# polarlightman/Scoring-rules-for-Gaussian-process-regression-a-new-approach-to-inference

Hardware: AMD Instinct MI355X
Metric: GP fit+predict+CRPS wall-clock (ms) at n=20k full / n=40k FITC; HBM GB/s & MFMA% (higher is better)
Workload: dtype f64; 1 GPU; C3 full GP fit(NLML+LOO-CRPS+LOO-LogS)+predict+score; n=20000, d=8, n_test=5000, kernel=ARD, parallelism=single

## Files before the change

include/gpscore.h:

```cpp
#ifndef GPSCORE_H
#define GPSCORE_H

#include <stdint.h>

#ifdef __cplusplus
extern "C" {
#endif

typedef struct gps_ctx gps_ctx;

enum { GPS_ARD = 0, GPS_RBF = 1 };
enum { GPS_FULL = 0, GPS_LOWER = 1 };

enum {
  GPS_OBJ_NLML = 0,
  GPS_OBJ_LOO_CRPS = 1,
  GPS_OBJ_LOO_LOGS = 2,
  GPS_OBJ_LOGDET = 3,
  GPS_OBJ_QUAD = 4,
  GPS_N_OBJ = 5
};
enum {
  GPS_SC_CRPS = 0, GPS_SC_LOGS = 1, GPS_SC_MSLL = 2, GPS_SC_SMSE = 3,
  GPS_SC_MSE = 4, GPS_SC_COVER = 5, GPS_N_SC = 6
// ... 13 lines not shown
  GPS_OPT_OVERLAP = 0,
  GPS_OPT_GEMM_MAP = 3,
  GPS_OPT_TINY_GEMM = 7,
  GPS_OPT_GRAM_REG = 9,
  GPS_OPT_GRAPH = 10,
  GPS_OPT_PRED_PRE = 11,
  GPS_OPT_DAG = 12,
  GPS_OPT_AR_CHUNKS = 15,
  GPS_OPT_DAG_TILES = 13,
  GPS_OPT_STREAM_K = 18,
  GPS_OPT_DAG_WGS = 19,
  GPS_OPT_DAG_GROUP = 17,
  GPS_OPT_SLAB_XCD = 26,
  GPS_OPT_DAG_ORDER = 25,
  GPS_OPT_FITC_DEP = 27,
};
int gps_ctx_set_option(gps_ctx* ctx, int key, int value);

enum { GPS_STAT_GRAPHS = 0, GPS_STAT_GRAPH_CAP = 1, GPS_STAT_GRAPH_OVERFLOW = 2,
       GPS_STAT_DEVICE_BYTES = 3, GPS_STAT_GRAPH_DROPPED = 4, GPS_STAT_GRAPH_EVICTED = 5,
       GPS_N_STATS = 6 };
int gps_ctx_stats(gps_ctx* ctx, int64_t* out, int cap);

int gps_dag_task_list(int T, int flags, uint32_t* out, int cap);

typedef struct gps_gemm_desc {
  int32_t lay_a, lay_b, epi;
  int32_t M, N, K;
  int64_t lda, ldb, ldc;
  double alpha, beta;
  int32_t tri, tri_off;
  int32_t lower_out, mirror;
  int32_t kend;
  int32_t tile, ksplit, map_mode;
  int32_t use_ws, sk_alone, dep_mode;
  int32_t reserved;
  int64_t ld_out, c_kslice_stride;
} gps_gemm_desc;
enum { GPS_GEMM_PLAN_TILE = 0, GPS_GEMM_PLAN_KSPLIT = 1, GPS_GEMM_PLAN_MAP = 2,
// ... 178 lines not shown
```

scoring-rules-for-gaussian-process-regression-a-new-approach-to-inference_amd/csrc/api.hip:

```cpp
#include "api_internal.h"

namespace gpsapi {

thread_local std::string g_err;

int fail(gps_ctx* ctx, int code, const std::string& msg) {
  if (ctx) ctx->err = msg;
  g_err = msg;
  return code;
}

hipError_t sync_ctx_streams(gps_ctx* ctx) {
  for (hipStream_t st : {ctx->stream, ctx->side, ctx->aux[0], ctx->aux[1]})
    if (st) {
      const hipError_t e = hipStreamSynchronize(st);
      if (e != hipSuccess) return e;
    }
  return hipSuccess;
}

hipError_t drop_graphs_in(gps_ctx* ctx, const void* p, size_t bytes) {
  if (!ctx || !p || ctx->pgraphs.empty()) return hipSuccess;
  const uintptr_t lo = (uintptr_t)p, hi = lo + bytes;
  bool synced = false;
// ... 200 lines not shown

int fitc_rowsq_dep(gps_ctx* ctx, const double* L, int* sig, int64_t ncols, int mode,
                   hipStream_t st, int64_t nb_dag) {
  const int64_t np = ctx->fn_pad, mp = ctx->m_pad;
  GemmParams p = gp0();
  p.A = ctx->Knm.d(); p.lda = mp; p.B = L; p.ldb = mp;
  p.M = (int)np; p.N = (int)ncols; p.K = (int)ncols; p.tri = TRI_K_LE_J;
  p.kend = (int)pad_to(ctx->m, 16);
  p.out0 = ctx->fslab.d(); p.ld_out = np;
  p.dep_sig = sig; p.dep_q = sig + kSigQueue; p.dep_err = static_cast<int*>(ctx->info.p) + 1;
  p.dep_grid = dag_width(ctx, nb_dag, true); p.dep_mode = mode;
  return gemm(ctx, LAY_N, LAY_T, EPI_ROWSQ, p, st);
}

int dag_list_key(const gps_ctx* ctx, int64_t nb) {
  return (int)(3 * nb + ctx->dag_order);
}

bool dag_block(const gps_ctx* ctx, int64_t nb) { return ctx->dag && nb >= 2 && nb <= ctx->dag_tiles; }

void dag_blocks(const gps_ctx* ctx, int64_t nb, std::vector<int>& sizes, int64_t& cnt) {
  if (nb <= 1) return;
  if (dag_block(ctx, nb)) {
    sizes.push_back((int)nb);
    cnt += dag_cnt_ints((int)nb);
    return;
  }
  dag_blocks(ctx, nb / 2, sizes, cnt);
  dag_blocks(ctx, nb - nb / 2, sizes, cnt);
}

int dag_width(const gps_ctx* ctx, int64_t nb, bool half) {
  const int auto_w = half ? std::max(4, ctx->ncu / 2) : ctx->ncu;
  return (int)std::min<int64_t>(ctx->dag_wgs > 0 ? ctx->dag_wgs : auto_w, std::max<int64_t>(4, 2 * nb * nb));
// ... 9 lines not shown
    ++ctx->fplan.leaves;
    return 0;
  }
  if (dag_block(ctx, nb)) {
    auto it = ctx->dag_lists.find(dag_list_key(ctx, nb));
    const int64_t need = dag_cnt_ints(nb);
    if (it == ctx->dag_lists.end() || ctx->dag_cnt_used + need > (int64_t)(ctx->dag_cnt.cap / 4))
      return fail(ctx, -2, "persistent factorisation: task list / counters not prepared");
    DagParams d;
    d.A = A; d.lda = lda; d.Linv = Linv; d.ldl = ldl; d.Lout = Lout; d.ldlo = ldlo;
    d.logdiag = logdiag; d.info = info; d.base = base; d.nreal = nreal; d.T = nb;
    d.tasks = static_cast<const uint32_t*>(it->second.first.p); d.ntasks = it->second.second;
    d.cnt = static_cast<int*>(ctx->dag_cnt.p) + ctx->dag_cnt_used;
    d.spin_ticks = 200000000ull;
    d.group = ctx->dag_group;
    d.sig = ctx->dag_sig;
    ctx->dag_sig = nullptr;
    ctx->dag_cnt_used += need;
    const double nn = 128.0 * nb;
    Prof pr(ctx, "potrf_dag", 2.0 * nn * nn * nn / 3.0, 0);
    HIPCHK(launch_potrf_dag(d, dag_width(ctx, nb, ctx->dag_half), s));
    gps_ctx::FactorPlan& fp = ctx->fplan;
    fp.dag_tmin = fp.dags ? std::min(fp.dag_tmin, nb) : nb;
    fp.dag_tmax = std::max(fp.dag_tmax, nb);
    ++fp.dags;
    return 0;
  }
  const int n1b = nb / 2, n2b = nb - n1b;
  const int n1 = n1b * GPS_TILE, n2 = n2b * GPS_TILE;
  double* A21 = A + (int64_t)n1 * lda;
// ... 115 lines not shown
bool factor_zeroed(const gps_ctx* ctx, const double* p, int64_t n_pad) {
  const auto it = ctx->zeroed.find((uintptr_t)p);
  return it != ctx->zeroed.end() && it->second == n_pad;
}

int potrf_inv(gps_ctx* ctx, double* A, int64_t n_pad, double* Linv, double* W, double* logdiag,
              int nreal, double* Lout) {
  if (!factor_zeroed(ctx, Linv, n_pad) || (Lout && !factor_zeroed(ctx, Lout, n_pad)))
    return fail(ctx, -1, "potrf_inv: factor buffer not zeroed for this size (internal contract)");
  std::vector<int> dsizes;
  int64_t dcnt = 0;
  dag_blocks(ctx, n_pad / GPS_TILE, dsizes, dcnt);
  for (int T : dsizes) {
    const int lk = dag_list_key(ctx, T);
    if (ctx->dag_lists.count(lk)) continue;
    const std::vector<uint32_t> tl = dag_task_list(T, ctx->dag_order, true);
    auto& e = ctx->dag_lists[lk];
    HIPCHK(ensure(ctx, e.first, tl.size() * 4));
    HIPCHK(hipMemcpyAsync(e.first.p, tl.data(), tl.size() * 4, hipMemcpyHostToDevice, ctx->stream));
    HIPCHK(hipStreamSynchronize(ctx->stream));
    e.second = (int)tl.size();
  }
  if (dcnt && ctx->dag_cnt.cap < (size_t)dcnt * 4) {
    HIPCHK(hipStreamSynchronize(ctx->stream));
    HIPCHK(ensure(ctx, ctx->dag_cnt, std::max<size_t>((size_t)dcnt * 4, (size_t)1 << 20)));
    HIPCHK(hipMemsetAsync(ctx->dag_cnt.p, 0, ctx->dag_cnt.cap, ctx->stream));
    HIPCHK(hipStreamSynchronize(ctx->stream));
  }
  auto eager = [&]() {
    ctx->sync_used = 0;
    ctx->pre.join = nullptr;
// ... 3 lines not shown
                         static_cast<int*>(ctx->info.p), 0, nreal, Lout, n_pad, true);
  };
  if (!ctx->graphs || ctx->prof || n_pad <= GPS_TILE) return eager();
  HIPCHK(ensure(ctx, ctx->ws_main, (size_t)kSplitWsDoubles * 8));
  HIPCHK(ensure(ctx, ctx->ws_side, (size_t)kSplitWsDoubles * 8));
  const bool pre = ctx->pre.kind == PRE_FITC_Q;
  std::vector<uintptr_t> key = {
      (uintptr_t)A, (uintptr_t)n_pad, (uintptr_t)Linv, (uintptr_t)W, (uintptr_t)logdiag,
      (uintptr_t)nreal, (uintptr_t)Lout, (uintptr_t)ctx->stream, (uintptr_t)ctx->side,
      (uintptr_t)ctx->overlap, (uintptr_t)ctx->gemm_map,
      (uintptr_t)g_tiny_gemm, (uintptr_t)g_stream_k, (uintptr_t)g_slab_xcd, (uintptr_t)ctx->info.p, (uintptr_t)ctx->ws_main.p,
      (uintptr_t)ctx->ws_side.p, (uintptr_t)pre,
      pre ? (uintptr_t)ctx->pre.n1 : 0, pre ? (uintptr_t)ctx->aux[0] : 0,
      pre ? (uintptr_t)ctx->Knm.p : 0, pre ? (uintptr_t)ctx->fslab.p : 0,
      pre ? (uintptr_t)ctx->fn_pad : 0, pre ? (uintptr_t)ctx->m_pad : 0, pre ? (uintptr_t)ctx->pre.sig : 0,
      (uintptr_t)ctx->dag, (uintptr_t)ctx->dag_tiles, (uintptr_t)ctx->dag_group, (uintptr_t)ctx->dag_wgs, (uintptr_t)ctx->dag_half,
      (uintptr_t)ctx->dag_cnt.p, (uintptr_t)ctx->sk_cnt.p, (uintptr_t)ctx->dag_sig};
  for (int T : dsizes) key.push_back((uintptr_t)ctx->dag_lists[dag_list_key(ctx, T)].first.p);
  for (auto& g : ctx->pgraphs)
    if (g.key == key) {
      g.last_use = ++ctx->graph_tick;
      HIPCHK(hipGraphLaunch(g.exec, ctx->stream));
      ctx->fplan = g.plan;
      ctx->fplan.replayed = 1;
      return 0;
    }
  if (ctx->pgraphs.size() >= kMaxGraphs) {
    size_t lru = 0;
    for (size_t i = 1; i < ctx->pgraphs.size(); ++i)
      if (ctx->pgraphs[i].last_use < ctx->pgraphs[lru].last_use) lru = i;
    HIPCHK(sync_ctx_streams(ctx));
// ... 225 lines not shown
      ctx->dag_wgs = value;
      return 0;
    case GPS_OPT_FITC_DEP: ctx->fitc_dep = value != 0; return 0;
    case GPS_OPT_DAG_ORDER:
      ARGCHK(value >= 0 && value <= 2, "GPS_OPT_DAG_ORDER must be 0, 1 or 2");
      ctx->dag_order = value;
      return 0;
    case GPS_OPT_DAG_GROUP:
      ARGCHK(value >= 2 && value <= 4, "GPS_OPT_DAG_GROUP must be 2, 3 or 4");
      ctx->dag_group = value;
      return 0;
    case GPS_OPT_DAG_TILES:
      ARGCHK(value >= 2 && value <= 64, "GPS_OPT_DAG_TILES must be in 2..64");
      ctx->dag_tiles = value;
      return 0;
    default: return fail(ctx, -1, "unknown option");
  }
}

void* gps_ctx_stream(gps_ctx* ctx) { return ctx ? (void*)ctx->stream : nullptr; }

int gps_ctx_synchronize(gps_ctx* ctx) {
  if (int rc = bind(ctx)) return rc;
  HIPCHK(hipStreamSynchronize(ctx->stream));
  return 0;
}

int gps_ctx_stats(gps_ctx* ctx, int64_t* out, int cap) {
  if (int rc = bind(ctx)) return rc;
  ARGCHK(out != nullptr && cap >= 0, "out is NULL or cap < 0");
  size_t bytes = 0;
  for (DBuf* b : ctx_buffers(ctx)) bytes += b->cap;
  int64_t v[GPS_N_STATS];
  v[GPS_STAT_GRAPHS] = (int64_t)ctx->pgraphs.size();
  v[GPS_STAT_GRAPH_CAP] = (int64_t)kMaxGraphs;
  v[GPS_STAT_GRAPH_OVERFLOW] = ctx->graph_overflow;
  v[GPS_STAT_GRAPH_DROPPED] = ctx->graph_dropped;
  v[GPS_STAT_GRAPH_EVICTED] = ctx->graph_evicted;
  v[GPS_STAT_DEVICE_BYTES] = (int64_t)bytes;
  for (int i = 0; i < cap && i < GPS_N_STATS; ++i) out[i] = v[i];
  return GPS_N_STATS;
}

int gps_dag_task_list(int T, int flags, uint32_t* out, int cap) {
  if (T < 2 || T > 64 || cap < 0 || (cap > 0 && !out) || (flags & ~13))
    return fail(nullptr, -1, "bad arguments");
  const std::vector<uint32_t> tl = dag_task_list(T, (flags >> 2 & 3) == 0 ? 1 : (flags >> 2 & 3) == 3 ? 0 : flags >> 2 & 3,
                                                 (flags & 1) != 0);
  for (int i = 0; i < cap && i < (int)tl.size(); ++i) out[i] = tl[i];
  return (int)tl.size();
}

int gps_phase_enable(gps_ctx* ctx, int on) {
  if (int rc = bind(ctx)) return rc;
  ctx->phase = on != 0;
  return 0;
}

int gps_phase_collect(gps_ctx* ctx, char* json_out, int64_t cap) {
  if (int rc = bind(ctx)) return rc;
  HIPCHK(sync_ctx_streams(ctx));
  std::map<std::string, std::pair<int, double>> agg;
  std::vector<std::string> order;
// ... 252 lines not shown
```

scoring-rules-for-gaussian-process-regression-a-new-approach-to-inference_amd/csrc/api_full.hip:

```cpp
#include "api_internal.h"

extern "C" {

int gps_full_set_data(gps_ctx* ctx, const double* X, const double* y, int64_t n, int d) {
  if (int rc = bind(ctx)) return rc;
  ARGCHK(X && y && n > 1 && d >= 1 && d <= GPS_MAX_D, "bad training data");
  ARGCHK(n <= (int64_t)1 << 30, "n too large");
  if (d != ctx->d) ctx->have_test = false;
  ctx->n = n;
  ctx->d = d;
  ctx->n_pad = pad_to(n);
  if (int rc = upload(ctx, ctx->X, X, n, d, ctx->n_pad)) return rc;
  if (int rc = upload(ctx, ctx->y, y, n, 1, ctx->n_pad)) return rc;
  double s = 0, s2 = 0;
  for (int64_t i = 0; i < n; ++i) s += y[i];
  const double mean = s / n;
  for (int64_t i = 0; i < n; ++i) s2 += (y[i] - mean) * (y[i] - mean);
  ctx->ytr_mean = mean;
  ctx->ytr_var = s2 / (n - 1);
  ctx->have_data = true;
  ctx->fitted = false;
  HIPCHK(hipStreamSynchronize(ctx->stream));
  return 0;
}
// ... 28 lines not shown
  }
  HIPCHK(ensure(ctx, ctx->W, potrf_ws_doubles(np) * 8));
  HIPCHK(ensure(ctx, ctx->logdiag, np * 8));
  HIPCHK(ensure(ctx, ctx->beta, np * 8));
  HIPCHK(ensure(ctx, ctx->alpha, np * 8));
  HIPCHK(ensure(ctx, ctx->dinv, np * 8));
  HIPCHK(ensure(ctx, ctx->mu_loo, np * 8));
  HIPCHK(ensure(ctx, ctx->var_loo, np * 8));
  const int64_t nchunk = (np + 255) / 256;
  HIPCHK(ensure(ctx, ctx->slab, (size_t)nchunk * np * 2 * 8));
  int rc;
  if ((rc = reset_info(ctx))) return rc;
  if ((rc = gram(ctx, "gram_kff", ctx->X.d(), (int)n, ctx->X.d(), (int)n, ctx->d, ctx->th,
                 ctx->th.sn2, 1, 1, ctx->A.d(), np, (int)np, (int)np)))
    return rc;
  if ((rc = potrf_inv(ctx, ctx->A.d(), np, ctx->Linv.d(), ctx->W.d(), ctx->logdiag.d(), (int)n,
                      nullptr)))
    return rc;
  {
    Prof pr(ctx, "gemv_beta", 0, 4.0 * (double)np * np);
    HIPCHK(launch_gemv_lower(ctx->Linv.d(), np, ctx->y.d(), ctx->beta.d(), (int)np, s));
  }
  int nchunk_c = 0;
  {
    Prof pr(ctx, "colred_alpha_dinv", 0, 4.0 * (double)np * np);
    nchunk_c = launch_colred_partials(ctx->Linv.d(), np, (int)np, (int)np, 1, ctx->beta.d(),
                                      ctx->slab.d(), s);
    ARGCHK(nchunk_c > 0, "column pass launch failed");
  }
  {
    double* part = row_part(ctx, np, 4);
    ARGCHK(part != nullptr, "out of device memory");
    Prof pr(ctx, "loo_finalize", 0, 0);
// ... 214 lines not shown
```

scoring-rules-for-gaussian-process-regression-a-new-approach-to-inference_amd/csrc/api_internal.h:

```cpp
#pragma once
#include <dlfcn.h>
#include <rccl/rccl.h>
#include <stdio.h>
#include <string.h>

#include <chrono>
#include <climits>
#include <cmath>
#include <condition_variable>
#include <map>
#include <memory>
#include <mutex>
#include <string>
#include <vector>

#include "gps_internal.h"
#include "gpscore.h"

using namespace gps;

namespace gpsapi {


struct DBuf {
// ... 66 lines not shown
  hipStream_t aux[2] = {nullptr, nullptr};
  bool overlap = true;
  int gemm_map = 0;
  int ar_chunks = 4;
  std::vector<hipEvent_t> ar_ev;
  int ncu = 0;
  std::vector<hipEvent_t> sync_ev;
  size_t sync_used = 0;
  bool graphs = true;
  bool pred_pre = true;
  bool dag = true;
  int dag_tiles = 20;
  int dag_group = 3;
  int dag_wgs = 0;
  int dag_order = 1;
  bool dag_half = false;
  bool fitc_dep = true;
  int* dag_sig = nullptr;
  DBuf dsig;
  std::map<int, std::pair<DBuf, int>> dag_lists;
  std::map<uintptr_t, int64_t> zeroed;
  DBuf dag_cnt;
  DBuf sk_cnt;
  int64_t dag_cnt_used = 0;
  struct PrePass {
    int kind = 0;
    int64_t n1 = 0;
    const double* L = nullptr;
    hipEvent_t join = nullptr;
    int* sig = nullptr;
// ... 139 lines not shown
void phase_mark(gps_ctx* c, const char* name);
hipEvent_t sync_event(gps_ctx* c);
GemmParams gp0();
const char* gemm_tag(int al, int bl, int epi, const GemmParams& p);
double gemm_flops(const GemmParams& p);
int gemm(gps_ctx* ctx, int al, int bl, int epi, const GemmParams& p, hipStream_t st = nullptr,
         GemmLaunchInfo* info = nullptr);
int gram(gps_ctx* ctx, const char* tag, const double* x, int n, const double* xp, int m, int d,
         const Theta& th, double diag_add, int lower, int pad_identity, double* out, int64_t ldo,
         int M, int N, hipStream_t st = nullptr);
int pred_rows(gps_ctx* ctx, int64_t r0, int64_t r1, const double* w, hipStream_t st);
int fitc_rowsq_cols(gps_ctx* ctx, const double* Lx, int64_t c0, int64_t c1, hipStream_t st);
int fitc_rowsq_dep(gps_ctx* ctx, const double* L, int* sig, int64_t ncols, int mode,
                   hipStream_t st, int64_t nb_dag);
int dag_list_key(const gps_ctx* ctx, int64_t nb);
bool dag_block(const gps_ctx* ctx, int64_t nb);
void dag_blocks(const gps_ctx* ctx, int64_t nb, std::vector<int>& sizes, int64_t& cnt);
int dag_width(const gps_ctx* ctx, int64_t nb, bool half);
int potrf_inv_rec(gps_ctx* ctx, double* A, int64_t lda, double* Linv, int64_t ldl, double* W,
                  int nb, double* logdiag, int* info, int base, int nreal, double* Lout,
                  int64_t ldlo, bool top = false);
size_t potrf_ws_doubles(int64_t n_pad);
int reset_info(gps_ctx* ctx);
hipError_t zero_factor(gps_ctx* ctx, double* p, int64_t n_pad, hipStream_t s);
bool factor_zeroed(const gps_ctx* ctx, const double* p, int64_t n_pad);
int potrf_inv(gps_ctx* ctx, double* A, int64_t n_pad, double* Linv, double* W, double* logdiag,
              int nreal, double* Lout);
int check_info(gps_ctx* ctx);
int set_theta(gps_ctx* ctx, Theta& th, int kind, const double* theta, int n_ell, int d);
int upload(gps_ctx* ctx, DBuf& b, const double* h, int64_t rows, int64_t cols, int64_t rows_pad);
// ... 32 lines not shown
```

scoring-rules-for-gaussian-process-regression-a-new-approach-to-inference_amd/csrc/gps_internal.h:

```cpp
#pragma once

#include <hip/hip_runtime.h>
#include <stdint.h>

#include <string>
#include <vector>

#define GPS_TILE 128
#define GPS_MAX_D 64

namespace gps {

inline int64_t pad_to(int64_t n, int64_t t = GPS_TILE) { return (n + t - 1) / t * t; }

struct GramParams {
  const double* x;
  const double* xp;
  double* out;
  int64_t ldo;
  int n, m;
  int M, N;
  int d;
  double sf2;
  double diag_add;
// ... 287 lines not shown
                             double* Lout, int64_t ldlo, double* logdiag, int* info,
                             int base, int n_real_in_block, hipStream_t s);

struct DagParams {
  double* A; int64_t lda;
  double* Linv; int64_t ldl;
  double* Lout; int64_t ldlo;
  double* logdiag; int* info; int base; int nreal;
  int T;
  const uint32_t* tasks; int ntasks;
  int* cnt;
  unsigned long long spin_ticks;
  unsigned long long* trace = nullptr;
  int group = 3;
  int* sig = nullptr;
};
hipError_t launch_potrf_dag(const DagParams& p, int nwg, hipStream_t s);
std::vector<uint32_t> dag_task_list(int T, int order = 1, bool fine = true);
inline int64_t dag_cnt_ints(int T) { return (16 + 2 * (int64_t)T * T + 63) / 64 * 64; }

hipError_t launch_gemv_lower(const double* L, int64_t ldl, const double* x, double* y,
                             int n_pad, hipStream_t s);
hipError_t launch_gemv_full(const double* M, int64_t ldm, const double* x, double* y,
                            int rows, int cols, hipStream_t s);
hipError_t launch_colred(const double* M, int64_t ldm, int rows, int cols, int lower,
                         const double* w, const double* rowscale, double* s1, double* s2,
                         double* slab, hipStream_t s, int crows = 256);
hipError_t launch_slab_sum(const double* slab, int64_t ld, int nslab, int64_t len,
                           const double* init, double* out, hipStream_t s);
hipError_t launch_sym_slab_sum(const double* slab, int64_t slice_stride, int nslab, int M,
                               const double* base, double* dst, hipStream_t s);

hipError_t launch_sym_pack(const double* slab, int64_t slice_stride, int nslab, int r0, int r1,
// ... 130 lines not shown
```

scoring-rules-for-gaussian-process-regression-a-new-approach-to-inference_amd/csrc/kernels_potrf.hip:

```cpp
#include <algorithm>
#include <queue>
#include <vector>

#include "gps_internal.h"

namespace gps {

namespace v4 {
typedef double d4 __attribute__((ext_vector_type(4)));
typedef double dv2 __attribute__((ext_vector_type(2)));
constexpr int TS = 17;
constexpr int TSZ = 16 * TS;
constexpr int NT = 36;
__device__ __forceinline__ constexpr int tix(int i, int j) { return i * (i + 1) / 2 + j; }

__device__ __forceinline__ double rl(double v, int lane) {
  const int lo = __builtin_amdgcn_readlane(__double2loint(v), lane);
  const int hi = __builtin_amdgcn_readlane(__double2hiint(v), lane);
  return __hiloint2double(hi, lo);
}
template <bool COH>
__device__ __forceinline__ void st_d(double* p, double v) {
  if constexpr (COH)
    __hip_atomic_store(reinterpret_cast<unsigned long long*>(p),
// ... 374 lines not shown
__device__ __forceinline__ double ld64(__amdgpu_buffer_rsrc_t r, uint32_t off) {
  return __builtin_bit_cast(double, __builtin_amdgcn_raw_buffer_load_b64(r, off, 0, AUX_SC1));
}
__device__ __forceinline__ void st64(__amdgpu_buffer_rsrc_t r, uint32_t off, double v) {
  __builtin_amdgcn_raw_buffer_store_b64(__builtin_bit_cast(v2u, v), r, off, 0, AUX_SC1);
}
__device__ __forceinline__ int ld_cnt(const int* p) {
  return __hip_atomic_load(p, __ATOMIC_RELAXED, __HIP_MEMORY_SCOPE_AGENT);
}

template <bool BT, int G>
__device__ __forceinline__ void wave_gemm32(const double* Ap, int64_t lda, const double* Bp,
                                            int64_t ldb, int kb, int ke, d4 (&acc)[2][2]) {
  const int lane = threadIdx.x & 63, r = lane & 15, g = lane >> 4;
  const __amdgpu_buffer_rsrc_t ra = rsrc(Ap, (uint32_t)(32 * lda * 8));
  const __amdgpu_buffer_rsrc_t rb = rsrc(Bp, (uint32_t)((BT ? 32 : 128) * ldb * 8));
  typedef double Frag[G][2][4];
  const int nc = (ke - kb) / 16;
  auto load_group = [&](int c, Frag& a, Frag& b) {
#pragma unroll
    for (int u = 0; u < G; ++u) {
      if (c + u >= nc) break;
      const int k = kb + 16 * (c + u) + 4 * g;
#pragma unroll
      for (int i = 0; i < 2; ++i) {
        const uint32_t oa = (uint32_t)(((int64_t)(16 * i + r) * lda + k) * 8);
        const dv2 a0 = ld128(ra, oa), a1 = ld128(ra, oa + 16);
        a[u][i][0] = a0.x; a[u][i][1] = a0.y; a[u][i][2] = a1.x; a[u][i][3] = a1.y;
        if constexpr (BT) {
          const uint32_t ob = (uint32_t)(((int64_t)(16 * i + r) * ldb + k) * 8);
          const dv2 b0 = ld128(rb, ob), b1 = ld128(rb, ob + 16);
// ... 200 lines not shown
      sh[1] = 0;
      sh[2] = (unsigned int)t;
    }
    __syncthreads();
    const unsigned int w = __builtin_amdgcn_readfirstlane(sh[0]);
    if (w == 0xffffffffu) break;
    if constexpr (TRACE) {
      trow = p.trace + 4 * (int64_t)__builtin_amdgcn_readfirstlane(sh[2]);
      if (tid == 0) {
        unsigned int xcc;
        asm volatile("s_getreg_b32 %0, hwreg(HW_REG_XCC_ID)" : "=s"(xcc));
        trow[0] = __builtin_amdgcn_s_memrealtime();
        trow[3] = (unsigned long long)blockIdx.x << 8 | (xcc & 15);
      }
    }
    const int type = w & 7, part = (w >> 3) & 15, fine = (w >> 7) & 1, ti = (w >> 8) & 255,
              tj = (w >> 16) & 255, tk = (w >> 24) & 255;
    if (wave == 0) {
      const int* c0 = nullptr; const int* c1 = nullptr; const int* c2 = nullptr;
      int v0 = 0, v1 = 0, v2 = 0;
      switch (type) {
        case 0:
          c0 = acnt + ti * T + ti; v0 = U * ti;
          break;
        case 1:
          c0 = acnt + ti * T + tk; v0 = U * tk;
          c1 = xcnt + tk * T + tk; v1 = 1;
          break;
        case 2:
          c0 = acnt + ti * T + tk; v0 = U * (tk + 1);
          c1 = acnt + tj * T + tk; v1 = U * (tk + 1);
          c2 = acnt + ti * T + tj; v2 = U * tk;
          break;
        case 3:
          c0 = acnt + ti * T + tj; v0 = U * (tj + 1);
          c1 = xcnt + tj * T + tk; v1 = tj == tk ? 1 : U * (tj - tk + 1);
          c2 = xcnt + ti * T + tk; v2 = U * (tj - tk);
          break;
        case 4:
          c0 = xcnt + ti * T + tk; v0 = U * (ti - tk);
          c1 = xcnt + ti * T + ti; v1 = 1;
          break;
        default: break;
      }
      if (!c1) { c1 = c0; v1 = v0; }
      if (!c2) { c2 = c0; v2 = v0; }
      constexpr unsigned int kMinPolls = 100000;
      unsigned long long t0 = __builtin_amdgcn_s_memrealtime();
      unsigned int ab = 0, polls = 0;
      int seen = -1;
      for (;;) {
        const int a0 = ld_cnt(c0), a1 = ld_cnt(c1), a2 = ld_cnt(c2), e = ld_cnt(err);
        if (__builtin_amdgcn_readfirstlane((a0 >= v0 && a1 >= v1 && a2 >= v2) ? 1 : 0)) break;
// ... 67 lines not shown
        case 1: {
          const int64_t K = 128 * (int64_t)tk;
          st.A = p.A + (R + q) * lda + K; st.lda = lda;
          st.B = p.Linv + (K + wv) * ldl + K; st.ldb = ldl; st.bt = 1;
          st.C = p.A + (R + q) * lda + K + wv; st.ldc = lda;
          if (p.Lout) { st.C2 = p.Lout + (R + q) * p.ldlo + K + wv; st.ldc2 = p.ldlo; }
          st.alpha = 1.0; st.beta = 0.0; st.kb = 0; st.ke = (int)wv + 32;
          out = acnt + ti * T + tk;
          break;
        }
        case 2: {
          const int64_t J = 128 * (int64_t)tj, K = 128 * (int64_t)tk;
          st.A = p.A + (R + q) * lda + K; st.lda = lda;
          st.B = p.A + (J + wv) * lda + K; st.ldb = lda; st.bt = 1;
          st.C = p.A + (R + q) * lda + J + wv; st.ldc = lda;
          st.alpha = -1.0; st.beta = 1.0; st.kb = 0; st.ke = 128;
          st.active = !(ti == tj && wave > part);
          out = acnt + ti * T + tj;
          break;
        }
        case 3: {
          const int64_t J = 128 * (int64_t)tj, K = 128 * (int64_t)tk;
          st.A = p.A + (R + q) * lda + J; st.lda = lda;
          st.B = p.Linv + J * ldl + K + wv; st.ldb = ldl; st.bt = 0;
          st.C = p.Linv + (R + q) * ldl + K + wv; st.ldc = ldl;
          st.alpha = 1.0; st.beta = tj == tk ? 0.0 : 1.0;
          st.kb = tj == tk ? (int)wv : 0; st.ke = 128;
          out = xcnt + ti * T + tk;
          break;
        }
        default: {
          const int64_t K = 128 * (int64_t)tk;
          st.A = p.Linv + (R + wv) * ldl + R; st.lda = ldl;
          st.B = p.Linv + R * ldl + K + q; st.ldb = ldl; st.bt = 0;
          st.C = p.Linv + (R + wv) * ldl + K + q; st.ldc = ldl;
          st.alpha = -1.0; st.beta = 0.0; st.kb = 0; st.ke = (int)wv + 32;
          out = xcnt + ti * T + tk;
          break;
        }
      }
      run_strip<G>(st);
    }
    asm volatile("s_waitcnt vmcnt(0)" ::: "memory");
// ... 15 lines not shown
      const int done = __hip_atomic_load(p.cnt + 2, __ATOMIC_RELAXED, __HIP_MEMORY_SCOPE_AGENT);
      const int e = __hip_atomic_load(err, __ATOMIC_RELAXED, __HIP_MEMORY_SCOPE_AGENT);
      if (e == 0x7f7f7f7f && (done != p.ntasks || head_end != p.ntasks + (int)gridDim.x))
        __hip_atomic_store(err, 2, __ATOMIC_RELAXED, __HIP_MEMORY_SCOPE_AGENT);
    }
    __syncthreads();
    const int n = 16 + 2 * T * T;
    for (int i = tid; i < n; i += 256)
      __hip_atomic_store(p.cnt + i, 0, __ATOMIC_RELAXED, __HIP_MEMORY_SCOPE_AGENT);
  }
}
}

hipError_t launch_potrf_dag(const DagParams& p, int nwg, hipStream_t s) {
  if ((p.lda & 1) || (p.ldl & 1) || (p.Lout && (p.ldlo & 1)) || p.T < 1 || p.T > 64 || nwg < 1 ||
      !p.tasks || !p.cnt || p.ntasks < 1)
    return hipErrorInvalidValue;
  if ((int64_t)128 * std::max(p.lda, p.ldl) * 8 >= ((int64_t)1 << 31)) return hipErrorInvalidValue;
  auto k = p.trace ? (p.group == 2 ? dag::potrf_dag_kernel<true, 2>
                                    : p.group == 3 ? dag::potrf_dag_kernel<true, 3> : dag::potrf_dag_kernel<true, 4>)
                   : (p.group == 2 ? dag::potrf_dag_kernel<false, 2>
                                    : p.group == 3 ? dag::potrf_dag_kernel<false, 3> : dag::potrf_dag_kernel<false, 4>);
  if (p.group < 2 || p.group > 4) return hipErrorInvalidValue;
  hipLaunchKernelGGL(k, dim3(nwg), dim3(256), 0, s, p);
  return hipGetLastError();
}

double g_dag_weights[7] = {35.0, 6.0, 9.7, 11.7, 11.2, 9.3, 2.5};

std::vector<uint32_t> dag_task_list(int T, int order, bool fine) {
  struct Task { int type, i, j, k; std::vector<int> deps; double est = 0.0, rank = 0.0; };
  auto is_fine = [&](const Task& t) {
    return fine && ((t.type == 1 && t.i == t.k + 1) || (t.type == 2 && t.i == t.k + 1 && t.j == t.i));
  };
  std::vector<Task> tk;
  std::vector<int> leaf(T), xkk(T), trsm(T * T, -1), fin(T * T, -1);
  std::vector<int> upd_last(T * T, -1), updx_last(T * T, -1);
  auto add = [&](int type, int i, int j, int k, std::vector<int> deps) {
    Task t;
    t.type = type; t.i = i; t.j = j; t.k = k;
    for (int d : deps)
      if (d >= 0) t.deps.push_back(d);
    tk.push_back(t);
    return (int)tk.size() - 1;
  };
  for (int k = 0; k < T; ++k) {
    leaf[k] = add(0, k, k, k, {upd_last[k * T + k]});
    xkk[k] = leaf[k];
    for (int i = k + 1; i < T; ++i) trsm[i * T + k] = add(1, i, k, k, {upd_last[i * T + k], xkk[k]});
    for (int j = k + 1; j < T; ++j)
      for (int i = j; i < T; ++i)
        upd_last[i * T + j] = add(2, i, j, k, {trsm[i * T + k], trsm[j * T + k], upd_last[i * T + j]});
  }
  auto xfinal = [&](int j, int k) { return j == k ? xkk[k] : fin[j * T + k]; };
  for (int j = 0; j < T; ++j) {
    for (int k = 0; k < j; ++k)
      fin[j * T + k] = add(4, j, k, k, {updx_last[j * T + k], xkk[j]});
    for (int i = j + 1; i < T; ++i)
      for (int k = 0; k <= j; ++k)
        updx_last[i * T + k] = add(3, i, j, k, {trsm[i * T + j], xfinal(j, k), updx_last[i * T + k]});
  }
  const int n = (int)tk.size();
  std::vector<std::vector<int>> succ(n);
  std::vector<int> indeg(n, 0);
  for (int t = 0; t < n; ++t)
    for (int d : tk[t].deps) { succ[d].push_back(t); ++indeg[t]; }
  if (order == 0) {
    auto dur = [&](const Task& t) { return t.type == 0 ? 36.0 : 4.0; };
    for (int t = 0; t < n; ++t)
      for (int d : tk[t].deps) tk[t].est = std::max(tk[t].est, tk[d].est + dur(tk[d]) + 3.0);
  } else if (order == 2) {
    auto dur = [&](const Task& t) {
      return t.type == 0 ? 38.0 : is_fine(t) ? 4.0 : 9.0;
    };
    for (int t = n - 1; t >= 0; --t) {
      double m = 0.0;
      for (int s2 : succ[t]) m = std::max(m, tk[s2].rank + 1.0);
      tk[t].rank = dur(tk[t]) + m;
      tk[t].est = -tk[t].rank;
    }
  } else {
    const double* w = g_dag_weights;
    auto dur = [&](const Task& t) {
      if (is_fine(t)) return w[1];
      switch (t.type) {
        case 0: return w[0];
        case 1: return w[2];
        case 2: return w[3];
        case 3: return w[4];
        default: return w[5];
      }
    };
    for (int t = n - 1; t >= 0; --t) {
      double m = 0.0;
      for (int s2 : succ[t]) m = std::max(m, tk[s2].rank + w[6]);
      tk[t].rank = dur(tk[t]) + m;
      tk[t].est = -tk[t].rank;
    }
  }
  std::priority_queue<std::pair<double, int>, std::vector<std::pair<double, int>>,
                      std::greater<std::pair<double, int>>> ready;
  for (int t = 0; t < n; ++t)
    if (!indeg[t]) ready.push({tk[t].est, t});
  std::vector<uint32_t> out;
  while (!ready.empty()) {
    const int t = ready.top().second;
    ready.pop();
    const Task& x = tk[t];
    const bool f = is_fine(x);
    const int parts = x.type == 0 ? 1 : !f ? dag::NP : x.type == 1 ? dag::NPF_TRSM : dag::NPF_UPD;
    for (int q = 0; q < parts; ++q)
      out.push_back((uint32_t)x.type | (uint32_t)q << 3 | (uint32_t)f << 7 | (uint32_t)x.i << 8 |
                    (uint32_t)x.j << 16 | (uint32_t)x.k << 24);
    for (int s2 : succ[t])
      if (!--indeg[s2]) ready.push({tk[s2].est, s2});
  }
  return out;
}

hipError_t launch_potrf_leaf(const double* A, int64_t lda, double* Linv, int64_t ldl, double* Lout,
                             int64_t ldlo, double* logdiag, int* info, int base, int nreal,
                             hipStream_t s) {
  if ((lda & 1) || (ldl & 1) || (Lout && (ldlo & 1))) return hipErrorInvalidValue;
  hipLaunchKernelGGL(v4::potrf_leaf_v4_kernel, dim3(1), dim3(256), 0, s, A, lda, Linv, ldl, Lout,
                     ldlo, logdiag, info, base, nreal);
  return hipGetLastError();
}

// ... 2 lines not shown
```

scoring-rules-for-gaussian-process-regression-a-new-approach-to-inference_amd/gpscore/_lib.py:

```python
from __future__ import annotations

import ctypes
import os

import numpy as np

_HERE = os.path.dirname(os.path.abspath(__file__))
LIB_PATH = os.environ.get("GPSCORE_LIB", os.path.join(_HERE, "libgpscore.so"))
ABI_VERSION = 900
GPS_N_STATS = 6
GPS_COMM_NONE, GPS_COMM_RCCL, GPS_COMM_LOCAL = 0, 1, 2
COMM_KINDS = {GPS_COMM_NONE: "none", GPS_COMM_RCCL: "rccl", GPS_COMM_LOCAL: "local"}

GPS_ARD, GPS_RBF = 0, 1
GPS_FULL, GPS_LOWER = 0, 1
GPS_OPT_OVERLAP, GPS_OPT_GEMM_MAP, GPS_OPT_TINY_GEMM, GPS_OPT_GRAM_REG = 0, 3, 7, 9
GPS_OPT_GRAPH = 10
GPS_OPT_PRED_PRE = 11
GPS_OPT_DAG = 12
GPS_OPT_DAG_TILES = 13
GPS_OPT_DAG_GROUP = 17
GPS_OPT_STREAM_K = 18
GPS_OPT_DAG_WGS = 19
GPS_OPT_DAG_ORDER = 25
GPS_OPT_SLAB_XCD = 26
GPS_OPT_FITC_DEP = 27
GPS_OPT_AR_CHUNKS = 15
OBJ_NAMES = ("nlml", "loo_crps", "loo_logs", "logdet", "quad")
SURFACE_NAMES = ("loo_crps", "insample_crps", "nlml", "loo_logs")
GPS_SURF_LOGS_ADD_NOISE = 1
GPS_BATCH_STALE_NOISE = 1
BATCH_MAX_N, BATCH_MAX_D = 128, 16
BATCH_FITC_MAX_M = 32
BATCH_FITC_TALL_MAX_N = 2048
BATCH_FULL_TALL_MAX_N = 512
SCORE_NAMES = ("test_crps", "test_logs", "test_msll", "test_smse", "test_mse", "test_cover")

_c_int, _c_i64, _c_dbl, _c_vp, _c_cp = (ctypes.c_int, ctypes.c_int64, ctypes.c_double,
                                        ctypes.c_void_p, ctypes.c_char_p)
_P = ctypes.POINTER(ctypes.c_double)

# ... 20 lines not shown
POTRF_PLAN_NAMES = ("n_pad", "leaves", "dags", "dag_tmin", "dag_tmax", "gemms", "replayed",
                    "reserved")

SIGNATURES = {
    "gps_version": (_c_int, []),
    "gps_build_id": (_c_int, [_c_cp, _c_int]),
    "gps_ctx_create": (_c_int, [_c_int, ctypes.POINTER(_c_vp)]),
    "gps_ctx_destroy": (_c_int, [_c_vp]),
    "gps_last_error": (_c_cp, [_c_vp]),
    "gps_ctx_set_stream": (_c_int, [_c_vp, _c_vp]),
    "gps_ctx_stream": (_c_vp, [_c_vp]),
    "gps_ctx_synchronize": (_c_int, [_c_vp]),
    "gps_ctx_set_option": (_c_int, [_c_vp, _c_int, _c_int]),
    "gps_ctx_stats": (_c_int, [_c_vp, _c_vp, _c_int]),
    "gps_dag_task_list": (_c_int, [_c_int, _c_int, _c_vp, _c_int]),
    "gps_gemm_diag_check": (_c_int, [ctypes.POINTER(GemmDesc), _c_int, _c_int, _c_int, _PI, _c_int,
                                     _c_int]),
    "gps_gemm_schedule": (_c_i64, [ctypes.POINTER(GemmDesc), _PI, _c_int, _c_int, _PI, _PI, _c_i64]),
    "gps_gemm_diag": (_c_int, [_c_vp, ctypes.POINTER(GemmDesc), _P, _P, _P, _P, _P, _PI, _P, _P,
                               _PI]),
    "gps_potrf_diag": (_c_int, [_c_vp, _c_i64, _P, _c_i64, _P, _P, _P, _PI, _PI]),
    "gps_grad_terms_diag": (_c_int, [_c_vp, _c_int, _c_int, _c_i64, _c_i64, _c_i64, _c_dbl, _PP,
                                     _PP]),
    "gps_grad_contract_diag": (_c_int, [_c_vp, _c_i64, _c_int, _P, _P, _c_dbl, _P, _P, _c_i64, _P,
                                        _P, _P, _P]),
    "gps_fitc_contract_diag": (_c_int, [_c_vp, _c_i64, _c_i64, _c_i64, _c_int, _P, _P, _P, _c_dbl,
                                        _c_int, _PP, _PI64, _P, _PP, _P, _PP, _PP, _P, _P]),
    "gps_prof_enable": (_c_int, [_c_vp, _c_int]),
    "gps_prof_collect": (_c_int, [_c_vp, _c_cp, _c_i64]),
    "gps_phase_enable": (_c_int, [_c_vp, _c_int]),
# ... 346 lines not shown
```

Baseline: 8.036 fit+predict+score units/s (C3 full GP, whole job).

## Batch DAG update tasks over multiple k-panels and raise DAG tile cap for full GP

Adds k-batching to the persistent Cholesky/inverse DAG. Runs of up to 8 consecutive rank-128 trailing updates (and Linv updates) fold into one task with a longer K loop, which cuts task count, dependency counter traffic and C read/write round-trips. For the full-GP fit, a separate tile cap (40) lets larger matrices run as a single DAG rather than recursive splits. With the 256 flag, batching applies only above the normal tile cap, so existing FITC sizes are unchanged. The trade-off is coarser tasks with more dependencies, which may reduce parallelism on the critical path, and the task encoding narrows tile indices to 6 bits.

```diff
diff --git a/include/gpscore.h b/include/gpscore.h
--- a/include/gpscore.h
+++ b/include/gpscore.h
@@ -51,6 +51,8 @@
   GPS_OPT_SLAB_XCD = 26,
   GPS_OPT_DAG_ORDER = 25,
   GPS_OPT_FITC_DEP = 27,
+  GPS_OPT_DAG_TILES_FULL = 28,
+  GPS_OPT_DAG_KBATCH = 29,
 };
 int gps_ctx_set_option(gps_ctx* ctx, int key, int value);
 
@@ -60,6 +62,7 @@
 int gps_ctx_stats(gps_ctx* ctx, int64_t* out, int cap);
 
 int gps_dag_task_list(int T, int flags, uint32_t* out, int cap);
+int gps_dag_task_list_ex(int T, int flags, int kb, int kg, uint32_t* out, int cap);
 
 typedef struct gps_gemm_desc {
   int32_t lay_a, lay_b, epi;
diff --git a/scoring-rules-for-gaussian-process-regression-a-new-approach-to-inference_amd/csrc/api.hip b/scoring-rules-for-gaussian-process-regression-a-new-approach-to-inference_amd/csrc/api.hip
--- a/scoring-rules-for-gaussian-process-regression-a-new-approach-to-inference_amd/csrc/api.hip
+++ b/scoring-rules-for-gaussian-process-regression-a-new-approach-to-inference_amd/csrc/api.hip
@@ -238,10 +238,18 @@
 }
 
 int dag_list_key(const gps_ctx* ctx, int64_t nb) {
-  return (int)(3 * nb + ctx->dag_order);
-}
-
-bool dag_block(const gps_ctx* ctx, int64_t nb) { return ctx->dag && nb >= 2 && nb <= ctx->dag_tiles; }
+  return (int)(3 * nb + ctx->dag_order) << 8 | dag_kg(ctx, nb) << 4 | dag_kb(ctx, nb);
+}
+int dag_kb(const gps_ctx* ctx, int64_t nb) {
+  if ((ctx->dag_kbatch & 256) && nb <= ctx->dag_tiles) return 1;
+  return std::max(1, ctx->dag_kbatch & 15);
+}
+int dag_kg(const gps_ctx* ctx, int64_t nb) { return dag_kb(ctx, nb) > 1 ? ctx->dag_kbatch >> 4 & 3 : 0; }
+
+bool dag_block(const gps_ctx* ctx, int64_t nb) {
+  const int cap = ctx->dag_full && ctx->dag_tiles_full ? ctx->dag_tiles_full : ctx->dag_tiles;
+  return ctx->dag && nb >= 2 && nb <= cap;
+}
 
 void dag_blocks(const gps_ctx* ctx, int64_t nb, std::vector<int>& sizes, int64_t& cnt) {
   if (nb <= 1) return;
@@ -281,6 +289,7 @@
     d.cnt = static_cast<int*>(ctx->dag_cnt.p) + ctx->dag_cnt_used;
     d.spin_ticks = 200000000ull;
     d.group = ctx->dag_group;
+    d.kbatch = dag_kb(ctx, nb);
     d.sig = ctx->dag_sig;
     ctx->dag_sig = nullptr;
     ctx->dag_cnt_used += need;
@@ -426,7 +435,7 @@
   for (int T : dsizes) {
     const int lk = dag_list_key(ctx, T);
     if (ctx->dag_lists.count(lk)) continue;
-    const std::vector<uint32_t> tl = dag_task_list(T, ctx->dag_order, true);
+    const std::vector<uint32_t> tl = dag_task_list(T, ctx->dag_order, true, dag_kb(ctx, T), dag_kg(ctx, T));
     auto& e = ctx->dag_lists[lk];
     HIPCHK(ensure(ctx, e.first, tl.size() * 4));
     HIPCHK(hipMemcpyAsync(e.first.p, tl.data(), tl.size() * 4, hipMemcpyHostToDevice, ctx->stream));
@@ -460,7 +469,8 @@
       pre ? (uintptr_t)ctx->pre.n1 : 0, pre ? (uintptr_t)ctx->aux[0] : 0,
       pre ? (uintptr_t)ctx->Knm.p : 0, pre ? (uintptr_t)ctx->fslab.p : 0,
       pre ? (uintptr_t)ctx->fn_pad : 0, pre ? (uintptr_t)ctx->m_pad : 0, pre ? (uintptr_t)ctx->pre.sig : 0,
-      (uintptr_t)ctx->dag, (uintptr_t)ctx->dag_tiles, (uintptr_t)ctx->dag_group, (uintptr_t)ctx->dag_wgs, (uintptr_t)ctx->dag_half,
+      (uintptr_t)ctx->dag, (uintptr_t)ctx->dag_tiles,
+      (uintptr_t)(ctx->dag_full ? ctx->dag_tiles_full : 0), (uintptr_t)ctx->dag_kbatch, (uintptr_t)ctx->dag_group, (uintptr_t)ctx->dag_wgs, (uintptr_t)ctx->dag_half,
       (uintptr_t)ctx->dag_cnt.p, (uintptr_t)ctx->sk_cnt.p, (uintptr_t)ctx->dag_sig};
   for (int T : dsizes) key.push_back((uintptr_t)ctx->dag_lists[dag_list_key(ctx, T)].first.p);
   for (auto& g : ctx->pgraphs)
@@ -716,6 +726,15 @@
       ARGCHK(value >= 2 && value <= 64, "GPS_OPT_DAG_TILES must be in 2..64");
       ctx->dag_tiles = value;
       return 0;
+    case GPS_OPT_DAG_TILES_FULL:
+      ARGCHK(value == 0 || (value >= 2 && value <= 64), "GPS_OPT_DAG_TILES_FULL must be 0 or in 2..64");
+      ctx->dag_tiles_full = value;
+      return 0;
+    case GPS_OPT_DAG_KBATCH:
+      ARGCHK(value >= 0 && (value & 15) <= 8 && (value >> 4 & 15) <= 3 && (value >> 9) == 0,
+             "GPS_OPT_DAG_KBATCH must be B | g << 4 [| 256] with B in 0..8 and g in 0..3");
+      ctx->dag_kbatch = (value & 15) < 2 ? 0 : value;
+      return 0;
     default: return fail(ctx, -1, "unknown option");
   }
 }
@@ -745,10 +764,14 @@
 }
 
 int gps_dag_task_list(int T, int flags, uint32_t* out, int cap) {
-  if (T < 2 || T > 64 || cap < 0 || (cap > 0 && !out) || (flags & ~13))
+  return gps_dag_task_list_ex(T, flags, 1, 0, out, cap);
+}
+
+int gps_dag_task_list_ex(int T, int flags, int kb, int kg, uint32_t* out, int cap) {
+  if (T < 2 || T > 64 || cap < 0 || (cap > 0 && !out) || (flags & ~13) || kb < 1 || kb > 8 || kg < 0 || kg > 3)
     return fail(nullptr, -1, "bad arguments");
   const std::vector<uint32_t> tl = dag_task_list(T, (flags >> 2 & 3) == 0 ? 1 : (flags >> 2 & 3) == 3 ? 0 : flags >> 2 & 3,
-                                                 (flags & 1) != 0);
+                                                 (flags & 1) != 0, kb, kg);
   for (int i = 0; i < cap && i < (int)tl.size(); ++i) out[i] = tl[i];
   return (int)tl.size();
 }
diff --git a/scoring-rules-for-gaussian-process-regression-a-new-approach-to-inference_amd/csrc/api_full.hip b/scoring-rules-for-gaussian-process-regression-a-new-approach-to-inference_amd/csrc/api_full.hip
--- a/scoring-rules-for-gaussian-process-regression-a-new-approach-to-inference_amd/csrc/api_full.hip
+++ b/scoring-rules-for-gaussian-process-regression-a-new-approach-to-inference_amd/csrc/api_full.hip
@@ -66,9 +66,10 @@
   if ((rc = gram(ctx, "gram_kff", ctx->X.d(), (int)n, ctx->X.d(), (int)n, ctx->d, ctx->th,
                  ctx->th.sn2, 1, 1, ctx->A.d(), np, (int)np, (int)np)))
     return rc;
-  if ((rc = potrf_inv(ctx, ctx->A.d(), np, ctx->Linv.d(), ctx->W.d(), ctx->logdiag.d(), (int)n,
-                      nullptr)))
-    return rc;
+  ctx->dag_full = true;
+  rc = potrf_inv(ctx, ctx->A.d(), np, ctx->Linv.d(), ctx->W.d(), ctx->logdiag.d(), (int)n, nullptr);
+  ctx->dag_full = false;
+  if (rc) return rc;
   {
     Prof pr(ctx, "gemv_beta", 0, 4.0 * (double)np * np);
     HIPCHK(launch_gemv_lower(ctx->Linv.d(), np, ctx->y.d(), ctx->beta.d(), (int)np, s));
diff --git a/scoring-rules-for-gaussian-process-regression-a-new-approach-to-inference_amd/csrc/api_internal.h b/scoring-rules-for-gaussian-process-regression-a-new-approach-to-inference_amd/csrc/api_internal.h
--- a/scoring-rules-for-gaussian-process-regression-a-new-approach-to-inference_amd/csrc/api_internal.h
+++ b/scoring-rules-for-gaussian-process-regression-a-new-approach-to-inference_amd/csrc/api_internal.h
@@ -104,6 +104,9 @@
   int dag_group = 3;
   int dag_wgs = 0;
   int dag_order = 1;
+  int dag_tiles_full = 40;
+  int dag_kbatch = 8 | 256;
+  bool dag_full = false;
   bool dag_half = false;
   bool fitc_dep = true;
   int* dag_sig = nullptr;
@@ -273,6 +276,8 @@
 int fitc_rowsq_dep(gps_ctx* ctx, const double* L, int* sig, int64_t ncols, int mode,
                    hipStream_t st, int64_t nb_dag);
 int dag_list_key(const gps_ctx* ctx, int64_t nb);
+int dag_kb(const gps_ctx* ctx, int64_t nb);
+int dag_kg(const gps_ctx* ctx, int64_t nb);
 bool dag_block(const gps_ctx* ctx, int64_t nb);
 void dag_blocks(const gps_ctx* ctx, int64_t nb, std::vector<int>& sizes, int64_t& cnt);
 int dag_width(const gps_ctx* ctx, int64_t nb, bool half);
diff --git a/scoring-rules-for-gaussian-process-regression-a-new-approach-to-inference_amd/csrc/gps_internal.h b/scoring-rules-for-gaussian-process-regression-a-new-approach-to-inference_amd/csrc/gps_internal.h
--- a/scoring-rules-for-gaussian-process-regression-a-new-approach-to-inference_amd/csrc/gps_internal.h
+++ b/scoring-rules-for-gaussian-process-regression-a-new-approach-to-inference_amd/csrc/gps_internal.h
@@ -325,9 +325,10 @@
   unsigned long long* trace = nullptr;
   int group = 3;
   int* sig = nullptr;
+  int kbatch = 1;
 };
 hipError_t launch_potrf_dag(const DagParams& p, int nwg, hipStream_t s);
-std::vector<uint32_t> dag_task_list(int T, int order = 1, bool fine = true);
+std::vector<uint32_t> dag_task_list(int T, int order = 1, bool fine = true, int kb = 1, int kg = 0);
 inline int64_t dag_cnt_ints(int T) { return (16 + 2 * (int64_t)T * T + 63) / 64 * 64; }
 
 hipError_t launch_gemv_lower(const double* L, int64_t ldl, const double* x, double* y,
diff --git a/scoring-rules-for-gaussian-process-regression-a-new-approach-to-inference_amd/csrc/kernels_potrf.hip b/scoring-rules-for-gaussian-process-regression-a-new-approach-to-inference_amd/csrc/kernels_potrf.hip
--- a/scoring-rules-for-gaussian-process-regression-a-new-approach-to-inference_amd/csrc/kernels_potrf.hip
+++ b/scoring-rules-for-gaussian-process-regression-a-new-approach-to-inference_amd/csrc/kernels_potrf.hip
@@ -412,7 +412,7 @@
                                             int64_t ldb, int kb, int ke, d4 (&acc)[2][2]) {
   const int lane = threadIdx.x & 63, r = lane & 15, g = lane >> 4;
   const __amdgpu_buffer_rsrc_t ra = rsrc(Ap, (uint32_t)(32 * lda * 8));
-  const __amdgpu_buffer_rsrc_t rb = rsrc(Bp, (uint32_t)((BT ? 32 : 128) * ldb * 8));
+  const __amdgpu_buffer_rsrc_t rb = rsrc(Bp, (uint32_t)((BT ? 32 : ke > 128 ? ke : 128) * ldb * 8));
   typedef double Frag[G][2][4];
   const int nc = (ke - kb) / 16;
   auto load_group = [&](int c, Frag& a, Frag& b) {
@@ -643,8 +643,9 @@
         trow[3] = (unsigned long long)blockIdx.x << 8 | (xcc & 15);
       }
     }
-    const int type = w & 7, part = (w >> 3) & 15, fine = (w >> 7) & 1, ti = (w >> 8) & 255,
-              tj = (w >> 16) & 255, tk = (w >> 24) & 255;
+    const int type = w & 7, part = (w >> 3) & 15, fine = (w >> 7) & 1, ti = (w >> 8) & 63,
+              tj = (w >> 16) & 63, tk = (w >> 24) & 63;
+    const int len = 1 + (int)((w >> 14) & 3) + 4 * (int)((w >> 22) & 1);
     if (wave == 0) {
       const int* c0 = nullptr; const int* c1 = nullptr; const int* c2 = nullptr;
       int v0 = 0, v1 = 0, v2 = 0;
@@ -656,16 +657,20 @@
           c0 = acnt + ti * T + tk; v0 = U * tk;
           c1 = xcnt + tk * T + tk; v1 = 1;
           break;
-        case 2:
-          c0 = acnt + ti * T + tk; v0 = U * (tk + 1);
-          c1 = acnt + tj * T + tk; v1 = U * (tk + 1);
+        case 2: {
+          const int kl = tk + len - 1;
+          c0 = acnt + ti * T + kl; v0 = U * (kl + 1);
+          c1 = acnt + tj * T + kl; v1 = U * (kl + 1);
           c2 = acnt + ti * T + tj; v2 = U * tk;
           break;
-        case 3:
-          c0 = acnt + ti * T + tj; v0 = U * (tj + 1);
-          c1 = xcnt + tj * T + tk; v1 = tj == tk ? 1 : U * (tj - tk + 1);
+        }
+        case 3: {
+          const int jl = tj + len - 1;
+          c0 = acnt + ti * T + jl; v0 = U * (jl + 1);
+          c1 = xcnt + jl * T + tk; v1 = jl == tk ? 1 : U * (jl - tk + 1);
           c2 = xcnt + ti * T + tk; v2 = U * (tj - tk);
           break;
+        }
         case 4:
           c0 = xcnt + ti * T + tk; v0 = U * (ti - tk);
           c1 = xcnt + ti * T + ti; v1 = 1;
@@ -763,9 +768,10 @@
           st.A = p.A + (R + q) * lda + K; st.lda = lda;
           st.B = p.A + (J + wv) * lda + K; st.ldb = lda; st.bt = 1;
           st.C = p.A + (R + q) * lda + J + wv; st.ldc = lda;
-          st.alpha = -1.0; st.beta = 1.0; st.kb = 0; st.ke = 128;
+          st.alpha = -1.0; st.beta = 1.0; st.kb = 0; st.ke = 128 * len;
           st.active = !(ti == tj && wave > part);
           out = acnt + ti * T + tj;
+          inc = len * (U / NP);
           break;
         }
         case 3: {
@@ -774,8 +780,9 @@
           st.B = p.Linv + J * ldl + K + wv; st.ldb = ldl; st.bt = 0;
           st.C = p.Linv + (R + q) * ldl + K + wv; st.ldc = ldl;
           st.alpha = 1.0; st.beta = tj == tk ? 0.0 : 1.0;
-          st.kb = tj == tk ? (int)wv : 0; st.ke = 128;
+          st.kb = tj == tk ? (int)wv : 0; st.ke = 128 * len;
           out = xcnt + ti * T + tk;
+          inc = len * (U / NP);
           break;
         }
         default: {
@@ -821,9 +828,9 @@
 
 hipError_t launch_potrf_dag(const DagParams& p, int nwg, hipStream_t s) {
   if ((p.lda & 1) || (p.ldl & 1) || (p.Lout && (p.ldlo & 1)) || p.T < 1 || p.T > 64 || nwg < 1 ||
-      !p.tasks || !p.cnt || p.ntasks < 1)
+      !p.tasks || !p.cnt || p.ntasks < 1 || p.kbatch < 1 || p.kbatch > 8)
     return hipErrorInvalidValue;
-  if ((int64_t)128 * std::max(p.lda, p.ldl) * 8 >= ((int64_t)1 << 31)) return hipErrorInvalidValue;
+  if ((int64_t)128 * p.kbatch * std::max(p.lda, p.ldl) * 8 >= ((int64_t)1 << 31)) return hipErrorInvalidValue;
   auto k = p.trace ? (p.group == 2 ? dag::potrf_dag_kernel<true, 2>
                                     : p.group == 3 ? dag::potrf_dag_kernel<true, 3> : dag::potrf_dag_kernel<true, 4>)
                    : (p.group == 2 ? dag::potrf_dag_kernel<false, 2>
@@ -835,37 +842,57 @@
 
 double g_dag_weights[7] = {35.0, 6.0, 9.7, 11.7, 11.2, 9.3, 2.5};
 
-std::vector<uint32_t> dag_task_list(int T, int order, bool fine) {
-  struct Task { int type, i, j, k; std::vector<int> deps; double est = 0.0, rank = 0.0; };
+std::vector<uint32_t> dag_task_list(int T, int order, bool fine, int kb, int kg) {
+  struct Task { int type, i, j, k, len; std::vector<int> deps; double est = 0.0, rank = 0.0; };
   auto is_fine = [&](const Task& t) {
     return fine && ((t.type == 1 && t.i == t.k + 1) || (t.type == 2 && t.i == t.k + 1 && t.j == t.i));
+  };
+  auto batch_of = [&](int t, int nt, int keep, int& b0, int& b1) {
+    const int nbat = kb > 1 ? std::max(0, nt - keep) : 0;
+    if (t >= nbat) { b0 = t; b1 = t + 1; return; }
+    b0 = t / kb * kb;
+    b1 = std::min(b0 + kb, nbat);
   };
   std::vector<Task> tk;
   std::vector<int> leaf(T), xkk(T), trsm(T * T, -1), fin(T * T, -1);
   std::vector<int> upd_last(T * T, -1), updx_last(T * T, -1);
-  auto add = [&](int type, int i, int j, int k, std::vector<int> deps) {
+  auto add = [&](int type, int i, int j, int k, int len, std::vector<int> deps) {
     Task t;
-    t.type = type; t.i = i; t.j = j; t.k = k;
+    t.type = type; t.i = i; t.j = j; t.k = k; t.len = len;
     for (int d : deps)
       if (d >= 0) t.deps.push_back(d);
     tk.push_back(t);
     return (int)tk.size() - 1;
   };
   for (int k = 0; k < T; ++k) {
-    leaf[k] = add(0, k, k, k, {upd_last[k * T + k]});
+    leaf[k] = add(0, k, k, k, 1, {upd_last[k * T + k]});
     xkk[k] = leaf[k];
-    for (int i = k + 1; i < T; ++i) trsm[i * T + k] = add(1, i, k, k, {upd_last[i * T + k], xkk[k]});
+    for (int i = k + 1; i < T; ++i) trsm[i * T + k] = add(1, i, k, k, 1, {upd_last[i * T + k], xkk[k]});
     for (int j = k + 1; j < T; ++j)
-      for (int i = j; i < T; ++i)
-        upd_last[i * T + j] = add(2, i, j, k, {trsm[i * T + k], trsm[j * T + k], upd_last[i * T + j]});
+      for (int i = j; i < T; ++i) {
+        int b0, b1;
+        batch_of(k, j, std::max(kg, fine && i == j ? 1 : 0), b0, b1);
+        if (k != b1 - 1) continue;
+        std::vector<int> deps = {upd_last[i * T + j]};
+        for (int q = b0; q < b1; ++q) { deps.push_back(trsm[i * T + q]); deps.push_back(trsm[j * T + q]); }
+        if (b1 - b0 == 1) deps = {trsm[i * T + k], trsm[j * T + k], upd_last[i * T + j]};
+        upd_last[i * T + j] = add(2, i, j, b0, b1 - b0, deps);
+      }
   }
   auto xfinal = [&](int j, int k) { return j == k ? xkk[k] : fin[j * T + k]; };
   for (int j = 0; j < T; ++j) {
     for (int k = 0; k < j; ++k)
-      fin[j * T + k] = add(4, j, k, k, {updx_last[j * T + k], xkk[j]});
+      fin[j * T + k] = add(4, j, k, k, 1, {updx_last[j * T + k], xkk[j]});
     for (int i = j + 1; i < T; ++i)
-      for (int k = 0; k <= j; ++k)
-        updx_last[i * T + k] = add(3, i, j, k, {trsm[i * T + j], xfinal(j, k), updx_last[i * T + k]});
+      for (int k = 0; k <= j; ++k) {
+        int b0, b1;
+        batch_of(j - k, i - k, kg, b0, b1);
+        if (j - k != b1 - 1) continue;
+        std::vector<int> deps = {updx_last[i * T + k]};
+        for (int q = b0 + k; q < b1 + k; ++q) { deps.push_back(trsm[i * T + q]); deps.push_back(xfinal(q, k)); }
+        if (b1 - b0 == 1) deps = {trsm[i * T + j], xfinal(j, k), updx_last[i * T + k]};
+        updx_last[i * T + k] = add(3, i, b0 + k, k, b1 - b0, deps);
+      }
   }
   const int n = (int)tk.size();
   std::vector<std::vector<int>> succ(n);
@@ -873,12 +900,12 @@
   for (int t = 0; t < n; ++t)
     for (int d : tk[t].deps) { succ[d].push_back(t); ++indeg[t]; }
   if (order == 0) {
-    auto dur = [&](const Task& t) { return t.type == 0 ? 36.0 : 4.0; };
+    auto dur = [&](const Task& t) { return t.type == 0 ? 36.0 : 4.0 * t.len; };
     for (int t = 0; t < n; ++t)
       for (int d : tk[t].deps) tk[t].est = std::max(tk[t].est, tk[d].est + dur(tk[d]) + 3.0);
   } else if (order == 2) {
     auto dur = [&](const Task& t) {
-      return t.type == 0 ? 38.0 : is_fine(t) ? 4.0 : 9.0;
+      return t.type == 0 ? 38.0 : is_fine(t) ? 4.0 : 9.0 * t.len;
     };
     for (int t = n - 1; t >= 0; --t) {
       double m = 0.0;
@@ -893,8 +920,8 @@
       switch (t.type) {
         case 0: return w[0];
         case 1: return w[2];
-        case 2: return w[3];
-        case 3: return w[4];
+        case 2: return w[3] * t.len;
+        case 3: return w[4] * t.len;
         default: return w[5];
       }
     };
@@ -918,7 +945,8 @@
     const int parts = x.type == 0 ? 1 : !f ? dag::NP : x.type == 1 ? dag::NPF_TRSM : dag::NPF_UPD;
     for (int q = 0; q < parts; ++q)
       out.push_back((uint32_t)x.type | (uint32_t)q << 3 | (uint32_t)f << 7 | (uint32_t)x.i << 8 |
-                    (uint32_t)x.j << 16 | (uint32_t)x.k << 24);
+                    (uint32_t)((x.len - 1) & 3) << 14 | (uint32_t)x.j << 16 |
+                    (uint32_t)((x.len - 1) >> 2) << 22 | (uint32_t)x.k << 24);
     for (int s2 : succ[t])
       if (!--indeg[s2]) ready.push({tk[s2].est, s2});
   }
diff --git a/scoring-rules-for-gaussian-process-regression-a-new-approach-to-inference_amd/gpscore/_lib.py b/scoring-rules-for-gaussian-process-regression-a-new-approach-to-inference_amd/gpscore/_lib.py
--- a/scoring-rules-for-gaussian-process-regression-a-new-approach-to-inference_amd/gpscore/_lib.py
+++ b/scoring-rules-for-gaussian-process-regression-a-new-approach-to-inference_amd/gpscore/_lib.py
@@ -25,6 +25,10 @@
 GPS_OPT_DAG_ORDER = 25
 GPS_OPT_SLAB_XCD = 26
 GPS_OPT_FITC_DEP = 27
+GPS_OPT_DAG_TILES_FULL = 28
+GPS_OPT_DAG_KBATCH = 29
+DAG_TILES_FULL_DEFAULT = 40
+DAG_KBATCH_DEFAULT = 8 | 256
 GPS_OPT_AR_CHUNKS = 15
 OBJ_NAMES = ("nlml", "loo_crps", "loo_logs", "logdet", "quad")
 SURFACE_NAMES = ("loo_crps", "insample_crps", "nlml", "loo_logs")
@@ -75,6 +79,7 @@
     "gps_ctx_set_option": (_c_int, [_c_vp, _c_int, _c_int]),
     "gps_ctx_stats": (_c_int, [_c_vp, _c_vp, _c_int]),
     "gps_dag_task_list": (_c_int, [_c_int, _c_int, _c_vp, _c_int]),
+    "gps_dag_task_list_ex": (_c_int, [_c_int, _c_int, _c_int, _c_int, _c_vp, _c_int]),
     "gps_gemm_diag_check": (_c_int, [ctypes.POINTER(GemmDesc), _c_int, _c_int, _c_int, _PI, _c_int,
                                      _c_int]),
     "gps_gemm_schedule": (_c_i64, [ctypes.POINTER(GemmDesc), _PI, _c_int, _c_int, _PI, _PI, _c_i64]),
```

Result: faster. 8.151 fit+predict+score units/s (C3 full GP, whole job), median of 6 (+1.4%).
